# Eddie-Wang1120/Eddie-Wang-Hackathon2023

Hardware: AMD Instinct MI355X
Metric: decode tokens/s, whole job (encoder + cross-KV + language-ID + prefill + greedy decode), Whisper large-v2 int8 weight-only + int8 KV; rtf reported beside it (higher is better)
Workload: dtype f16

## Files before the change

### eddie-wang-hackathon2023_amd/csrc/attn_decode.hip

```cpp
#include <hip/hip_ext.h>

#include <atomic>

#include "common.h"
#include "kernels.h"

namespace wm {

constexpr float ATTN_SCALE = 0.35355339059327373f;
constexpr int MAX_L = 4;

template <bool I8>
__global__ __launch_bounds__(64) void attn_self_kernel(AttnSelfParams p) {
    __builtin_amdgcn_s_setprio(3);

    constexpr int MAXT = 512;
    __shared__ float s_p[MAXT];
    __shared__ h16 s_qall[MAX_L][64], s_knew[MAX_L][64], s_vnew[MAX_L][64];

    const int h = blockIdx.x, lane = threadIdx.x;
    int b = blockIdx.y;
    const int32_t* lsrc = p.live ? p.live : (const int32_t*)p.part;
    const int32_t live_n = lsrc[0], live_b = lsrc[p.live ? 1 + b : 0];
    const int32_t t_now = (p.t_dev ? p.t_dev : (const int32_t*)p.part)[0];
// ... 103 lines not shown
                            }
                        }
                    } else {
                        const half8v* kr = (const half8v*)(pastK + (size_t)j * 128);
#pragma unroll
                        for (int c = 0; c < 8; ++c) {
                            const half8v w = j0 == 0 ? __builtin_bit_cast(half8v, kpre[c]) : kr[c];
#pragma unroll
                            for (int e = 0; e < 8; ++e)
                                acc = fmaf((float)s_q[c * 8 + e], r16((float)w[e] * ATTN_SCALE), acc);
                        }
                    }
                } else {
                    const h16* kn = s_knew[j - T];
#pragma unroll 8
                    for (int e = 0; e < 64; ++e) acc = fmaf((float)s_q[e], r16((float)kn[e] * ATTN_SCALE), acc);
                }
                sc = r16(f32_as_is(acc));
            }
            if (j < MAXT) s_p[j] = sc;
            mx = fmaxf(mx, sc);
        }
        mx = wave_max_nomfma(mx);
        float sum = 0.f;
        __syncthreads();
        for (int j = lane; j < nk; j += 64) {
            const float e = __expf(s_p[j] - mx);
            s_p[j] = e;
            sum += e;
        }
        sum = wave_sum_nomfma(sum);
        const float inv = 1.0f / sum;
        __syncthreads();
        for (int j = lane; j < nk; j += 64) s_p[j] = r16(s_p[j] * inv);
        __syncthreads();
        float o = 0.f;
        int j = 0;
        if (I8) {
            const int8_t* pv = (const int8_t*)pastV + lane;
#pragma unroll
            for (int u = 0; u < 32; ++u)
                if (u < T) o = fmaf(s_p[u], r16((float)vpre8[u] * t_dq), o);
            j = min(T, 32);
            for (; j + 32 <= T; j += 32) {
                int8_t vq[32];
#pragma unroll
                for (int u = 0; u < 32; ++u) vq[u] = pv[(size_t)(j + u) * 64];
#pragma unroll
                for (int u = 0; u < 32; ++u) o = fmaf(s_p[j + u], r16((float)vq[u] * t_dq), o);
            }
            for (; j + 8 <= T; j += 8) {
                int8_t vq[8];
#pragma unroll
                for (int u = 0; u < 8; ++u) vq[u] = pv[(size_t)(j + u) * 64];
#pragma unroll
                for (int u = 0; u < 8; ++u) o = fmaf(s_p[j + u], r16((float)vq[u] * t_dq), o);
            }
            for (; j < T; ++j) o = fmaf(s_p[j], r16((float)pv[(size_t)j * 64] * t_dq), o);
        } else {
            const h16* pv = (const h16*)pastV + lane;
#pragma unroll
            for (int u = 0; u < 32; ++u)
                if (u < T) o = fmaf(s_p[u], (float)vpre16[u], o);
            j = min(T, 32);
            for (; j + 32 <= T; j += 32) {
                h16 vh[32];
#pragma unroll
                for (int u = 0; u < 32; ++u) vh[u] = pv[(size_t)(j + u) * 64];
#pragma unroll
                for (int u = 0; u < 32; ++u) o = fmaf(s_p[j + u], (float)vh[u], o);
            }
            for (; j + 8 <= T; j += 8) {
                h16 vh[8];
#pragma unroll
                for (int u = 0; u < 8; ++u) vh[u] = pv[(size_t)(j + u) * 64];
#pragma unroll
                for (int u = 0; u < 8; ++u) o = fmaf(s_p[j + u], (float)vh[u], o);
            }
            for (; j < T; ++j) o = fmaf(s_p[j], (float)pv[(size_t)j * 64], o);
        }
        for (; j < nk; ++j) o = fmaf(s_p[j], (float)s_vnew[j - T][lane], o);
        p.out[(size_t)(b * p.L + i) * p.ldo + h * 64 + lane] = (h16)f32_as_is(o);
        __syncthreads();
    }
}

constexpr int SELF_WAVES = 4;
template <bool I8>
__global__ __launch_bounds__(64 * SELF_WAVES) void attn_self_wg_kernel(AttnSelfParams p) {
    __builtin_amdgcn_s_setprio(3);
    constexpr int MAXT = 512;
    constexpr int ES = I8 ? 1 : 2;
    constexpr int ROW_B = 64 * ES;
    constexpr int DIMS = 16 / ES;
    constexpr int NCH = 64 / DIMS;
    constexpr int VROWS = 64 / NCH;
    constexpr int KCH = ROW_B / 16;
    constexpr int VPRE = 4;
    constexpr int NT = 64 * SELF_WAVES;
    __shared__ float s_p[MAXT];
    __shared__ h16 s_qall[MAX_L][64], s_knew[MAX_L][64], s_vnew[MAX_L][64];
    __shared__ float s_o[NT][DIMS + 1];
    __shared__ float s_red[2][SELF_WAVES];
    __shared__ float s_lut[I8 ? 512 + MAX_L * 64 : 1];

    const int h = blockIdx.x, tid = threadIdx.x, lane = tid & 63, wid = tid >> 6;
    int b = blockIdx.y;
    const int32_t* lsrc = p.live ? p.live : (const int32_t*)p.part;
    const int32_t live_n = lsrc[0], live_b = lsrc[p.live ? 1 + b : 0];
    const int32_t t_now = (p.t_dev ? p.t_dev : (const int32_t*)p.part)[0];
    if (p.live) {
        if (b >= live_n) return;
        b = live_b;
    }
    const int T = p.t_dev ? t_now : p.T;
    const int C = p.H * 64;
    const unsigned char* pastK = (const unsigned char*)p.past + ((size_t)b * p.past_bstride + (size_t)(0 * p.H + h) * p.past_cap * 64) * ES;
    const unsigned char* pastV = (const unsigned char*)p.past + ((size_t)b * p.past_bstride + (size_t)(1 * p.H + h) * p.past_cap * 64) * ES;
    const int vr = lane / NCH, vc = lane % NCH;
    uint4 kpre[KCH], vpre[VPRE];
    if (T > 0) {
        const int kr = min(64 * wid + lane, T - 1);
#pragma unroll
        for (int c = 0; c < KCH; ++c) kpre[c] = ((const uint4*)(pastK + (size_t)kr * ROW_B))[c];
#pragma unroll
        for (int n = 0; n < VPRE; ++n) {
            const int row = min((wid + SELF_WAVES * n) * VROWS + vr, T - 1);
            vpre[n] = *(const uint4*)(pastV + (size_t)row * ROW_B + vc * 16);
        }
    }
    const float t_dq = p.kv_scale;
    const float inv_t = 1.0f / p.kv_scale;
    if constexpr (I8) {
        const float d = r16((float)(int)(int8_t)(tid & 255) * t_dq);
        s_lut[tid & 255] = r16(d * ATTN_SCALE);
        s_lut[256 + (tid & 255)] = d;
    }
    const size_t sstride = p.part_sstride ? (size_t)p.part_sstride : (size_t)p.B * p.L * p.ldp;

    if (wid == 0) {
        for (int i = 0; i < p.L; ++i) {
            const int m = b * p.L + i;
            float q = 0.f, k = 0.f, v = 0.f;
            const h16* bsrc = p.bias ? p.bias + h * 64 + lane : (const h16*)p.part;
            const int bstep = p.bias ? C : 0;
            const h16 bq_raw = bsrc[0], bk_raw = bsrc[bstep], bv_raw = bsrc[2 * bstep];
            const float* row = p.part + (size_t)m * p.ldp + h * 64 + lane;
            int s = 0;
            for (; s + 4 <= p.ksplit; s += 4) {
                const float* r0 = row + (size_t)s * sstride;
                const float* r1 = r0 + sstride; const float* r2 = r1 + sstride; const float* r3 = r2 + sstride;
                const float q0 = r0[0], q1 = r1[0], q2 = r2[0], q3 = r3[0];
                const float k0 = r0[C], k1 = r1[C], k2 = r2[C], k3 = r3[C];
                const float v0 = r0[2 * C], v1 = r1[2 * C], v2 = r2[2 * C], v3 = r3[2 * C];
                q += (q0 + q1) + (q2 + q3); k += (k0 + k1) + (k2 + k3); v += (v0 + v1) + (v2 + v3);
            }
            for (; s < p.ksplit; ++s) {
                const float* r0 = row + (size_t)s * sstride;
                q += r0[0]; k += r0[C]; v += r0[2 * C];
            }
            q = r16(q + (p.bias ? (float)bq_raw : 0.f));
            k = r16(k + (p.bias ? (float)bk_raw : 0.f));
            v = r16(v + (p.bias ? (float)bv_raw : 0.f));
            if (p.amax) {
                const float a = wave_max_nomfma(fmaxf(fabsf(q), fmaxf(fabsf(k), fabsf(v))));
                if (lane == 0) atomicMax((unsigned int*)p.amax, __float_as_uint(a));
// ... 47 lines not shown
                            acc = fmaf((float)s_q[c * 16 + e], s_lut[idx], acc);
                        }
                    } else {
                        const half8v wh = __builtin_bit_cast(half8v, w);
                        const half8v kn8 = *(const half8v*)(&s_knew[jn][c * 8]);
#pragma unroll
                        for (int e = 0; e < 8; ++e) {
                            const float xk = cached ? (float)wh[e] : (float)kn8[e];
                            acc = fmaf((float)s_q[c * 8 + e], r16(xk * ATTN_SCALE), acc);
                        }
                    }
                }
                sc = r16(f32_as_is(acc));
                s_p[j] = sc;
            }
            mx = fmaxf(mx, sc);
        }
        mx = wave_max_nomfma(mx);
        if (lane == 0) s_red[0][wid] = mx;
        __syncthreads();
        mx = fmaxf(fmaxf(s_red[0][0], s_red[0][1]), fmaxf(s_red[0][2], s_red[0][3]));
        const float e0 = tid < nk ? __expf(s_p[tid] - mx) : 0.f;
        const float e1 = tid + NT < nk ? __expf(s_p[tid + NT] - mx) : 0.f;
        const float wsum = wave_sum_nomfma(e0 + e1);
        if (lane == 0) s_red[1][wid] = wsum;
        __syncthreads();
        const float inv = 1.0f / ((s_red[1][0] + s_red[1][1]) + (s_red[1][2] + s_red[1][3]));
        if (tid < nk) s_p[tid] = r16(e0 * inv);
        if (tid + NT < nk) s_p[tid + NT] = r16(e1 * inv);
        __syncthreads();
        float o[DIMS];
#pragma unroll
        for (int d = 0; d < DIMS; ++d) o[d] = 0.f;
        auto add_block = [&](int vb, const uint4& w) {
            const int row = vb * VROWS + vr;
            const float pj = row < T ? s_p[row] : 0.f;
            if (I8) {
                const uint32_t ws[4] = {w.x, w.y, w.z, w.w};
#pragma unroll
                for (int d = 0; d < 16; ++d)
                    o[d] = fmaf(pj, s_lut[256 + ((ws[d >> 2] >> (8 * (d & 3))) & 0xff)], o[d]);
            } else {
                const half8v wh = __builtin_bit_cast(half8v, w);
#pragma unroll
                for (int d = 0; d < 8; ++d) o[d] = fmaf(pj, (float)wh[d], o[d]);
            }
        };
#pragma unroll
        for (int n = 0; n < VPRE; ++n) {
            const int vb = wid + SELF_WAVES * n;
            if (vb * VROWS < T) add_block(vb, vpre[n]);
        }
        for (int vb = wid + SELF_WAVES * VPRE; vb * VROWS < T; vb += SELF_WAVES) {
            const int row = min(vb * VROWS + vr, T - 1);
            add_block(vb, *(const uint4*)(pastV + (size_t)row * ROW_B + vc * 16));
        }
#pragma unroll
        for (int d = 0; d < DIMS; ++d) s_o[tid][d] = o[d];
        __syncthreads();
        if (wid == 0) {
            const int ch = lane / DIMS, d = lane % DIMS;
            float part[SELF_WAVES][VROWS];
#pragma unroll
            for (int w = 0; w < SELF_WAVES; ++w)
#pragma unroll
                for (int r = 0; r < VROWS; ++r) part[w][r] = s_o[w * 64 + r * NCH + ch][d];
            float acc = 0.f;
#pragma unroll
            for (int w = 0; w < SELF_WAVES; ++w)
#pragma unroll
                for (int r = 0; r < VROWS; ++r) acc += part[w][r];
            for (int j = T; j < nk; ++j) acc = fmaf(s_p[j], (float)s_vnew[j - T][lane], acc);
            p.out[(size_t)(b * p.L + i) * p.ldo + h * 64 + lane] = (h16)f32_as_is(acc);
        }
        __syncthreads();
    }
}

int launch_attn_self(const AttnSelfParams& p, hipStream_t stream) {
    WM_REQUIRE(p.L >= 1 && p.L <= MAX_L, "attn_self: L=%d out of range [1,%d]", p.L, MAX_L);
    WM_REQUIRE(p.T + p.L <= 512, "attn_self: T+L=%d exceeds 512", p.T + p.L);
    WM_REQUIRE(p.T + p.L <= p.present_cap, "attn_self: present capacity %d < T+L=%d", p.present_cap, p.T + p.L);
    WM_REQUIRE(!p.int8_kv || p.kv_scale > 0.f, "attn_self: int8 KV needs a positive scale");
    WM_REQUIRE(p.waves == 0 || p.waves == 1 || p.waves == SELF_WAVES, "attn_self: waves=%d (0, 1 or %d)", p.waves, SELF_WAVES);
    if (p.waves == SELF_WAVES) {
        if (p.int8_kv) hipLaunchKernelGGL(attn_self_wg_kernel<true>, dim3(p.H, p.B), dim3(64 * SELF_WAVES), 0, stream, p);
        else hipLaunchKernelGGL(attn_self_wg_kernel<false>, dim3(p.H, p.B), dim3(64 * SELF_WAVES), 0, stream, p);
    } else if (p.int8_kv)
        hipLaunchKernelGGL(attn_self_kernel<true>, dim3(p.H, p.B), dim3(64), 0, stream, p);
    else
        hipLaunchKernelGGL(attn_self_kernel<false>, dim3(p.H, p.B), dim3(64), 0, stream, p);
    WM_LAUNCH_CHECK(stream, "attn_self");
    return 0;
}

constexpr int CROSS_MAX_KEYS = 1536;
constexpr int CROSS_MAX_SPLIT = 16;


template <int L, bool I8 = false, int UNR_ = 0, bool SKIP = false>
__global__ __launch_bounds__(256) void attn_cross_kernel(AttnCrossParams p) {
    constexpr int DPL = I8 ? 16 : 8;
    constexpr int LPR = 64 / DPL;
    constexpr int RPI = 64 / LPR;
    constexpr int ESZ = I8 ? 1 : 2;
#ifndef CROSS_UNR
#define CROSS_UNR 4
#endif
    constexpr int UNR = UNR_ > 0 ? UNR_ : CROSS_UNR;
    __shared__ float s_sc[L][CROSS_MAX_KEYS];
    __shared__ float s_red[L][4][2];
    __shared__ float s_o[4][L][64];
    __shared__ unsigned char s_live[SKIP ? CROSS_MAX_KEYS / 8 : 1];

    const int tid = threadIdx.x, lane = tid & 63, wid = __builtin_amdgcn_readfirstlane(tid >> 6);
    const int sub = lane % LPR, rowi = lane / LPR;
    const int per_split = (((p.Tk + p.nsplit - 1) / p.nsplit) + 7) & ~7;
    constexpr int STRIDE = 4 * RPI * UNR;
    const int first = wid * (RPI * UNR);
    const int n_rows = p.live ? p.live[0] : p.B;
    const int n_items = p.H * n_rows * p.nsplit;

    struct Item { int h, b, sp, k_begin, nkeys; const unsigned char* K; const unsigned char* V; };
    auto geometry = [&](int item) {
        Item it;
        it.h = item % p.H; it.b = (item / p.H) % n_rows; it.sp = item / (p.H * n_rows);
        if (p.live) it.b = p.live[1 + it.b];
        it.k_begin = it.sp * per_split;
        it.nkeys = max(0, min(p.Tk, it.k_begin + per_split) - it.k_begin);
        it.K = (const unsigned char*)p.kv + ((size_t)it.b * p.kv_bstride + ((size_t)(0 * p.H + it.h) * p.Tk) * 64) * ESZ;
        it.V = (const unsigned char*)p.kv + ((size_t)it.b * p.kv_bstride + ((size_t)(1 * p.H + it.h) * p.Tk) * 64) * ESZ;
        return it;
    };
    auto issue = [&](u32x4 (&dst)[UNR], const unsigned char* base, int k_begin, int nkeys, int r0) {
#pragma unroll
        for (int u = 0; u < UNR; ++u) {
            const int rr = min(r0 + u * RPI + rowi, nkeys - 1);
            dst[u] = __builtin_nontemporal_load((const u32x4*)(base + ((size_t)(k_begin + rr) * 64 + sub * DPL) * ESZ));
        }
        __builtin_amdgcn_sched_barrier(0);
    };

    auto pipeline = [&](u32x4 (&X)[UNR], u32x4 (&Y)[UNR], int nb, auto&& fetch, auto&& consume) {
        int k = 0;
        for (; k + 2 < nb; k += 2) {
            fetch(Y, k + 1);
            consume(X, k);
            fetch(X, k + 2);
            consume(Y, k + 1);
        }
        if (nb - k == 2) {
            fetch(Y, k + 1);
            consume(X, k);
            consume(Y, k + 1);
        } else {
            consume(X, k);
        }
    };
    for (int item = blockIdx.x; item < n_items; item += gridDim.x) {
    const Item it = geometry(item);
    const int h = it.h, b = it.b, sp = it.sp, k_begin = it.k_begin, nkeys = it.nkeys;
    if (nkeys == 0) {
        for (int idx = tid; idx < L * 66; idx += 256) {
            float* w = p.ws + ((((size_t)b * p.H + h) * p.nsplit + sp) * L) * 66;
            w[idx] = (idx % 66 == 0) ? -INFINITY : 0.f;
        }
        continue;
    }
    const unsigned char* K = it.K;
    const unsigned char* V = it.V;
    const int nb = (nkeys + STRIDE - 1) / STRIDE;
    u32x4 bufA[UNR], bufB[UNR];
    issue(bufA, K, k_begin, nkeys, first);

// ... 361 lines not shown
```

### eddie-wang-hackathon2023_amd/csrc/engine.hip

```cpp
#include <stdarg.h>
#include <stdio.h>
#include <stdlib.h>
#include <string.h>

#include <atomic>
#include <map>
#include <mutex>
#include <unordered_map>
#include <string>
#include <vector>

#include "../../include/whisper_mi355.h"
#include "common.h"
#include "kernels.h"

namespace wm {

static thread_local char g_err[1024] = "";
void set_error(const char* fmt, ...) {
    va_list ap;
    va_start(ap, fmt);
    vsnprintf(g_err, sizeof(g_err), fmt, ap);
    va_end(ap);
}
// ... 558 lines not shown
}
}

namespace { constexpr int DEC_CHUNK = 4; }

size_t wm_decoder_workspace_bytes(const wm_engine* e, int batch, int n_new) {
    if (!e || e->kind != WM_ENGINE_DECODER || batch < 1 || n_new < 1) return 0;
    if (n_new <= DEC_CHUNK) return carve_decoder(e, batch, n_new, nullptr).total;
    return carve_decoder(e, batch, DEC_CHUNK, nullptr).total + align_up((size_t)batch * DEC_CHUNK * e->dims.n_vocab * sizeof(h16));
}

namespace {
__global__ void stamp_kernel(long long* tl, int cap, long long tag, long long what) {
    if (threadIdx.x != 0) return;
    const int i = atomicAdd((int*)tl, 1);
    if (i < cap) { tl[1 + 3 * i] = tag; tl[2 + 3 * i] = what; tl[3 + 3 * i] = wall_clock64(); }
}

constexpr int SMALL_PATH_DEFAULT_ROWS = 16;
std::atomic<int> g_cross_v_skip{CROSS_V_SKIP_DEFAULT};
std::atomic<int> g_decode_chain{DECODE_CHAIN_DEFAULT};
struct ChainDev {
    std::mutex mu;
    int n_cu = 0;
    unsigned* err_host = nullptr; unsigned* err_dev = nullptr;
    bool declined = false; std::string reason, footprint;
    std::map<long long, bool> resident;
    std::atomic<long long> launches{0};
    std::atomic<long long> declined_calls{0};
};
ChainDev g_chain_dev[64];
static ChainDev& chain_dev_slot(int device) { return g_chain_dev[device >= 0 && device < 64 ? device : 0]; }
int chain_dev_init(ChainDev& cd, int device) {
    std::lock_guard<std::mutex> lk(cd.mu);
    if (cd.n_cu > 0 && cd.err_host) return 0;
    int v = 0;
    WM_CHECK_HIP(hipDeviceGetAttribute(&v, hipDeviceAttributeMultiprocessorCount, device));
    void* host = nullptr; void* dev = nullptr;
    WM_CHECK_HIP(hipHostMalloc(&host, 64, hipHostMallocMapped | hipHostMallocCoherent));
    memset(host, 0, 64);
    WM_CHECK_HIP(hipHostGetDevicePointer(&dev, host, 0));
    cd.err_host = (unsigned*)host; cd.err_dev = (unsigned*)dev;
    cd.n_cu = v > 0 ? v : 1;
    return 0;
}
inline unsigned chain_err_peek(const ChainDev& cd) {
    return cd.err_host ? __atomic_load_n(cd.err_host, __ATOMIC_RELAXED) : 0u;
}
bool stream_has_all_cus(hipStream_t s, int n_cu) {
    uint32_t mask[32];
    memset(mask, 0, sizeof(mask));
    if (hipExtStreamGetCUMask(s, 32, mask) != hipSuccess) { (void)hipGetLastError(); return true; }
    int bits = 0;
    for (uint32_t m : mask) bits += __builtin_popcount(m);
    return bits == 0 || bits >= n_cu;
}
std::atomic<int> g_small_rows{-1};
int small_path_max_rows() {
    int r = g_small_rows.load(std::memory_order_relaxed);
    if (r < 0) {
        r = lab_env_int("WM_SMALL_PATH", SMALL_PATH_DEFAULT_ROWS);
        r = r < 0 ? 0 : (r > GEMV_SMALL_MAX_M ? GEMV_SMALL_MAX_M : r);
        g_small_rows.store(r, std::memory_order_relaxed);
    }
    return r;
}

std::atomic<int> g_rows_min{-1};
int rows_path_min_rows() {
    int r = g_rows_min.load(std::memory_order_relaxed);
    if (r < 0) {
        r = lab_env_int("WM_ROWS_PATH", 1) == 0 ? 0 : lab_env_int("WM_ROWS_MIN", 40);
        if (r < 0) r = 0;
        g_rows_min.store(r, std::memory_order_relaxed);
    }
    return r;
}

std::atomic<int> g_self_waves{-1};
int self_attn_waves(int rows) {
    int w = g_self_waves.load(std::memory_order_relaxed);
    if (w < 0) {
        w = lab_env_int("WM_SELF_WAVES", 0);
        if (w != 1 && w != 4) w = 0;
        g_self_waves.store(w, std::memory_order_relaxed);
    }
    return w ? w : (rows <= small_path_max_rows() ? 4 : 1);
}

int chain_max_rows() {
    static const int r = [] { const int v = lab_env_int("WM_CHAIN_ROWS", CHAIN_MAX_ROWS); return v < 1 ? 1 : (v > CHAIN_MAX_ROWS ? CHAIN_MAX_ROWS : v); }();
    return r;
}

struct GroupStep {
    const wm_engine* e; const wm_decoder_io* io; DecWs w;
    int B, L, T, C, H, M;
    bool small = false;
    bool chain = false;
    int chain_wgs = 0; unsigned* chain_err = nullptr; ChainDev* chain_cd = nullptr;
    bool rows = false;
    bool fused() const { return small || rows; }

    int gemv(const Lin& l, const h16* A, int lda, int mode, const h16* ln_g, const h16* ln_b, h16* out16, int ld16, hipStream_t s) {
        GemvSmallParams p{};
        p.A = A; p.lda = lda; p.M = M; p.K = l.K; p.Wt = l.w; p.n_blocks = l.n_blocks; p.w8 = l.wcode; p.scale = l.s;
        p.ln_g = ln_g; p.ln_b = ln_b;
        p.mode = mode; p.bias = l.b; p.gelu_kind = e->gelu();
        p.out32 = w.part; p.ld32 = l.N;
        p.out16 = out16; p.ld16 = ld16; p.n_valid = l.N;
        p.x = w.x; p.ldx = C;
        return small ? launch_gemv_small(p, s) : launch_gemm_rows(p, s);
    }

    Profiler* prof = nullptr;

    void mark(int layer, int pos, hipStream_t s) {
        static const bool fine = lab_env_int("WM_TIMELINE_FINE", 0) == 1;
        if (fine && prof->timeline)
            hipLaunchKernelGGL(stamp_kernel, dim3(1), dim3(64), 0, s, prof->timeline, prof->timeline_cap, (long long)(uintptr_t)io->logits, (long long)(1000 + 32 * layer + pos));
    }

    int init(const wm_engine* e_, const wm_decoder_io* io_, hipStream_t stream, bool alone = true) {
        e = e_; io = io_;
        prof = &g_prof_dev[e->device >= 0 && e->device < MAX_DEVICES ? e->device : 0];
        WM_REQUIRE(io && io->tokens && io->positional_embedding && io->present && io->cross && io->logits && io->workspace,
                   "wm_decoder_step: null argument");
        const wm_dims& d = e->dims;
        B = io->batch; L = io->n_new; T = io->n_past; C = d.n_text_state; H = d.n_text_head; M = B * L;
        WM_REQUIRE(B >= 1 && L >= 1 && L <= 4 && T >= 0, "wm_decoder_step: bad batch/n_new/n_past (%d, %d, %d)", B, L, T);
        WM_REQUIRE(T + L <= d.n_text_ctx, "wm_decoder_step: T+L=%d exceeds n_text_ctx=%d", T + L, d.n_text_ctx);
        WM_REQUIRE(T == 0 || io->past, "wm_decoder_step: n_past > 0 needs past buffers");
        WM_REQUIRE(T == 0 || io->past_capacity >= T, "wm_decoder_step: past capacity %d < n_past %d", io->past_capacity, T);
        WM_REQUIRE(io->present_capacity >= T + L, "wm_decoder_step: present capacity %d < n_past + n_new = %d", io->present_capacity, T + L);
        WM_REQUIRE(!io->n_past_dev || (L == 1 && io->past), "wm_decoder_step: a device step counter needs n_new == 1 and past buffers");
        WM_REQUIRE(C == H * 64, "head size must be 64");
        w = carve_decoder(e, B, L, io->workspace);
        WM_REQUIRE(io->workspace_bytes >= w.total, "decoder workspace too small: %zu < %zu", io->workspace_bytes, w.total);
        small = M <= small_path_max_rows();
        rows = !small && rows_path_min_rows() > 0 && M >= rows_path_min_rows() && !e->dec.empty() && gemm_rows_supports(C, e->dec[0].qkv.wcode);
        chain = false;
        hipStreamCaptureStatus cap_st = hipStreamCaptureStatusNone;
        const bool capturing = hipStreamIsCapturing(stream, &cap_st) == hipSuccess && cap_st != hipStreamCaptureStatusNone;
        ChainDev& cd = chain_dev_slot(e->device);
        if (!capturing && chain_err_peek(cd) != 0) {
            set_error("wm_decoder_step: a one-launch decode step on device %d gave up waiting for its workgroups (they were not resident "
                      "together): the results since then are invalid.  Call wm_decode_chain_error() to acknowledge and decode again -- the device "
                      "takes the launch-per-kernel path from then on (wm_set_decode_chain re-arms the one-launch forms)", e->device);
            return 1;
        }
        if (alone && small && L == 1 && M <= chain_max_rows() && !e->dec.empty() && e->chain_dev && g_decode_chain.load(std::memory_order_relaxed) && !io->qkv_amax) {
            if (chain_dev_init(cd, e->device)) return 2;
            const int n_cu = cd.n_cu;
            chain_wgs = n_cu > 256 ? 256 : n_cu; chain_err = cd.err_dev; chain_cd = &cd;
            bool ok = gemv_chain_supports(C, e->dec[0].qkv.wcode, n_cu) && w.nsplit == 4 && !e->i8cross() && self_attn_waves(M) == 4 &&
                      io->present_capacity <= 512 && !(M > 2 && e->dec[0].qkv.wcode == 4) &&
                      (M > 4 ? (M * H <= chain_wgs && M * H * w.nsplit <= 4 * chain_wgs)
                             : M * H + (M > 2 ? (M * H * w.nsplit + 1) / 2 : M * H * w.nsplit) <= chain_wgs);
            for (int i = 0; ok && i < e->dims.n_text_layer; ++i)
                ok = io->present[i] && io->cross[i] &&
                     (T == 0 ? io->n_past_dev == nullptr : (io->past[i] == io->present[i] && io->past_capacity == io->present_capacity));
            if (ok) {
                std::lock_guard<std::mutex> lk(cd.mu);
                ok = !cd.declined;
                if (ok) {
                    const long long key = ((long long)M << 48) | ((long long)e->dec[0].qkv.wcode << 40) | ((long long)(e->i8kv() ? 1 : 0) << 32) | ((long long)e->dims.n_audio_ctx << 8) | w.nsplit;
                    auto it = cd.resident.find(key);
// ... 401 lines not shown
}

int wm_step_advance(int32_t* counter, wm_stream_t stream) { return launch_step_advance(counter, (hipStream_t)stream); }
int wm_step_finish(int32_t* counter, const int32_t* done, int batch, int32_t* live, wm_stream_t stream) {
    return launch_step_finish(counter, done, batch, live, (hipStream_t)stream);
}

int wm_gemm(const void* A, int lda, int M, int K, const void* W, int N, int w8, const void* scale,
            const void* bias, const void* residual, int ldr, int act, void* C, int ldc,
            void* workspace, size_t workspace_bytes, wm_stream_t stream) {
    GemmBigParams p{};
    p.A = (const h16*)A; p.lda = lda; p.M = M; p.K = K; p.W = W; p.N = N;
    p.bias = (const h16*)bias; p.C = (h16*)C; p.ldc = ldc;
    p.residual = (const h16*)residual; p.ldr = ldr; p.act = act;
    if (w8) {
        WM_REQUIRE(scale && workspace, "wm_gemm: int8 weights need their scales and a workspace for the fp16 expansion");
        WM_REQUIRE(workspace_bytes >= (size_t)N * K * sizeof(h16), "wm_gemm: workspace too small: %zu < %zu", workspace_bytes, (size_t)N * K * sizeof(h16));
        if (launch_dequant_w8((const int8_t*)W, (const h16*)scale, (h16*)workspace, N, K, (hipStream_t)stream)) return 2;
        p.W = workspace;
    }
    return launch_gemm_f16(p, (hipStream_t)stream);
}

int wm_conv1d_gelu(const void* x_pad, int B, int T_in, int C_in, const void* W, int K, const void* bias, int C_out,
                   int stride, int gelu, void* out, wm_stream_t stream) {
    WM_REQUIRE(x_pad && W && out && B >= 1 && T_in >= 1, "wm_conv1d_gelu: null argument or empty input");
    WM_REQUIRE(stride == 1 || stride == 2, "wm_conv1d_gelu: stride %d (1 or 2)", stride);
    WM_REQUIRE(T_in % stride == 0 && K >= 3 * C_in, "wm_conv1d_gelu: T_in=%d, K=%d < 3*C_in=%d", T_in, K, 3 * C_in);
    const int T_out = T_in / stride;
    GemmBigParams p{};
    p.A = (const h16*)x_pad; p.lda = stride * C_in; p.M = B * T_out; p.K = K; p.W = W; p.N = C_out;
    p.a_rows = T_out; p.a_bstride = (long)(T_in + 2) * C_in;
    p.bias = (const h16*)bias; p.C = (h16*)out; p.ldc = C_out; p.act = gelu;
    return launch_gemm_f16(p, (hipStream_t)stream);
}

int wm_argmax(const void* logits, int64_t row_stride, int batch, int n_vocab, int32_t* ids, wm_stream_t stream) {
    WM_REQUIRE(logits && ids && batch >= 1 && n_vocab >= 1, "wm_argmax: null argument or empty input");
    return launch_argmax((const h16*)logits, (long)row_stride, batch, n_vocab, ids, (hipStream_t)stream);
}

int wm_gemm_skinny(const void* A, int lda, int M, int K, const void* Wt, int n_blocks, int w8,
                   const void* scale, int ksplit, float* part, wm_stream_t stream) {
    GemmSkinnyParams p{};
    p.A = (const h16*)A; p.lda = lda; p.M = M; p.K = K; p.Wt = Wt; p.n_blocks = n_blocks; p.w8 = w8;
    p.scale = (const h16*)scale; p.ksplit = ksplit; p.part = part;
    return launch_gemm_skinny(p, (hipStream_t)stream);
}
int wm_gemm_skinny_default_ksplit(int M, int K, int n_blocks, int w8) { return skinny_default_ksplit(M, K, n_blocks, w8); }

int wm_set_rows_path(int min_rows) {
    const int prev = rows_path_min_rows();
    g_rows_min.store(min_rows < 0 ? 0 : min_rows, std::memory_order_relaxed);
    return prev;
}

int wm_gemm_rows(const wm_gemv_io* io, wm_stream_t stream) {
    WM_REQUIRE(io && io->a && io->wt, "wm_gemm_rows: null argument");
    GemvSmallParams p{};
    p.A = (const h16*)io->a; p.lda = io->lda; p.M = io->m; p.K = io->k; p.Wt = io->wt; p.n_blocks = io->n_blocks; p.w8 = io->w8;
    p.scale = (const h16*)io->scale;
    p.ln_g = (const h16*)io->ln_gamma; p.ln_b = (const h16*)io->ln_beta;
    p.mode = io->mode; p.bias = (const h16*)io->bias; p.gelu_kind = io->gelu_kind;
    p.out32 = io->out32; p.ld32 = io->ld32; p.out16 = (h16*)io->out16; p.ld16 = io->ld16; p.n_valid = io->n_valid;
    p.x = (h16*)io->x; p.ldx = io->ldx;
    return launch_gemm_rows(p, (hipStream_t)stream);
}

int wm_lab_knobs(char* buf, size_t cap) {
    std::lock_guard<std::mutex> lk(g_lab_mu);
    if (buf && cap > 0) { strncpy(buf, g_lab_honoured.c_str(), cap - 1); buf[cap - 1] = 0; }
    return (int)g_lab_honoured.size();
}

int wm_set_gemm_small_tiles(int tiles) {
    const int prev = get_gemm_small_tiles();
    set_gemm_small_tiles(tiles);
    return prev;
}

int wm_set_self_attn_waves(int waves) {
    self_attn_waves(1);
    const int prev = g_self_waves.load(std::memory_order_relaxed);
    g_self_waves.store(waves == 1 || waves == 4 ? waves : 0, std::memory_order_relaxed);
    return prev;
}

int wm_set_small_batch_rows(int rows) {
    const int prev = small_path_max_rows();
    g_small_rows.store(rows < 0 ? 0 : (rows > GEMV_SMALL_MAX_M ? GEMV_SMALL_MAX_M : rows), std::memory_order_relaxed);
    return prev;
}

int wm_gemv_fused(const wm_gemv_io* io, wm_stream_t stream) {
    WM_REQUIRE(io && io->a && io->wt, "wm_gemv_fused: null argument");
    GemvSmallParams p{};
    p.A = (const h16*)io->a; p.lda = io->lda; p.M = io->m; p.K = io->k; p.Wt = io->wt; p.n_blocks = io->n_blocks; p.w8 = io->w8;
    p.scale = (const h16*)io->scale;
    p.ln_g = (const h16*)io->ln_gamma; p.ln_b = (const h16*)io->ln_beta;
    p.mode = io->mode; p.bias = (const h16*)io->bias; p.gelu_kind = io->gelu_kind;
    p.out32 = io->out32; p.ld32 = io->ld32; p.out16 = (h16*)io->out16; p.ld16 = io->ld16; p.n_valid = io->n_valid;
    p.x = (h16*)io->x; p.ldx = io->ldx;
    return launch_gemv_small(p, (hipStream_t)stream);
}

int wm_layernorm(const void* x, int ldx, int M, int N, const void* gamma, const void* beta, void* out, int ldo,
                 wm_stream_t stream) {
    return launch_layernorm((const h16*)x, ldx, M, N, (const h16*)gamma, (const h16*)beta, (h16*)out, ldo, (hipStream_t)stream);
}

int wm_attn_encoder(const void* qkv, int ld, int B, int T, int H, void* out, int ldo, wm_stream_t stream) {
    AttnEncParams p{(const h16*)qkv, ld, B, T, H, (h16*)out, ldo};
    return launch_attn_encoder(p, (hipStream_t)stream);
}

int wm_attn_decode_cross(const float* q, int B, int L, int H, int Tk, const void* kv, void* out, int nsplit,
                         float* ws, wm_stream_t stream) {
    AttnCrossParams p{};
    p.part = q; p.ksplit = 1; p.ldp = H * 64; p.bias = nullptr;
    p.B = B; p.L = L; p.H = H; p.Tk = Tk; p.kv = (const h16*)kv; p.kv_bstride = (long)2 * H * Tk * 64;
    p.out = (h16*)out; p.ldo = H * 64; p.nsplit = nsplit; p.ws = ws;
    p.skip_zero_rows = g_cross_v_skip.load(std::memory_order_relaxed);
    return launch_attn_cross(p, (hipStream_t)stream);
}

int wm_set_decode_chain(int on) {
    const int prev = g_decode_chain.load(std::memory_order_relaxed);
    g_decode_chain.store(on < 0 ? DECODE_CHAIN_DEFAULT : (on > 2 ? 2 : on), std::memory_order_relaxed);
    for (ChainDev& cd : g_chain_dev) {
        std::lock_guard<std::mutex> lk(cd.mu);
        if (cd.declined) { cd.declined = false; cd.reason.clear(); }
    }
    return prev;
}

int wm_decode_chain_error(int* out) {
    WM_REQUIRE(out, "wm_decode_chain_error: null argument");
    ChainDev& cd = chain_dev_slot(current_device_index());
    const unsigned v = chain_err_peek(cd);
    *out = (int)v;
    if (v) {
        std::lock_guard<std::mutex> lk(cd.mu);
        __atomic_store_n(cd.err_host, 0u, __ATOMIC_RELAXED);
        cd.declined = true;
        cd.reason = "a one-launch decode step gave up waiting for its workgroups (they were not resident together)";
    }
    return 0;
}

int wm_decode_chain_status(wm_chain_status* out) {
    WM_REQUIRE(out, "wm_decode_chain_status: null argument");
    ChainDev& cd = chain_dev_slot(current_device_index());
    std::lock_guard<std::mutex> lk(cd.mu);
    memset(out, 0, sizeof(*out));
    out->mode = g_decode_chain.load(std::memory_order_relaxed);
    out->launches = cd.launches.load(std::memory_order_relaxed);
    out->declined_calls = cd.declined_calls.load(std::memory_order_relaxed);
    out->declined = cd.declined ? 1 : 0;
    out->error_pending = chain_err_peek(cd) ? 1 : 0;
    snprintf(out->reason, sizeof(out->reason), "%s", cd.reason.c_str());
    snprintf(out->footprint, sizeof(out->footprint), "%s", cd.footprint.c_str());
    return 0;
}

int wm_debug_occupy(int n_workgroups, size_t lds_bytes, int64_t microseconds, wm_stream_t stream) {
    return launch_occupy(n_workgroups, lds_bytes, (long long)microseconds, (hipStream_t)stream);
}
// ... 47 lines not shown
```

### eddie-wang-hackathon2023_amd/csrc/kernels.h

```cpp
#pragma once
#include "common.h"

namespace wm {

struct GemmBigParams {
    const h16* A; int lda; int M; int K;
    const void* W; int N;
    const h16* bias;
    h16* C; int ldc;
    const h16* residual; int ldr; int res_mod;
    int act;
    int colscale_n; float colscale;
    int out_mode;
    int hs_T, hs_H, hs_kv;
    float q8_inv_scale;
    int a_rows; long a_bstride;
    int c_rows; long c_bstride;
    int max_wgs;
    int nt_flags;
    int tile_rows;
};
int launch_gemm_f16(const GemmBigParams& p, hipStream_t stream);
constexpr int GEMM_SMALL_TILES_DEFAULT = 150;
constexpr int GEMM_TINY_TILES_DEFAULT = 160;
// ... 43 lines not shown
};
struct ChainLayerStatic { const h16* qkv_bias; const h16* cq_bias; float kv_scale; int pad_; };
struct ChainLayerIo { const void* cross_kv; void* cache; };
struct GemvChainParams {
    int n_stages; const ChainStage* st;
    float* out32;
    int w8, gelu_kind;
    h16* x;
    unsigned long long* gran_x; unsigned long long* gran_h;
    const h16* cross_kv; int cross_Tk, cross_heads, cross_nsplit; const h16* cross_qbias;
    unsigned long long* gran_q;
    int cross_at, merge_at, merge_nsplit, merge_heads;
    unsigned long long* gran_p;
    const float* self_part; const h16* self_bias; void* self_cache; int self_cap, self_T, self_heads, self_i8; const int32_t* self_t_dev;
    float self_kv_scale; h16* self_out; unsigned long long* gran_c;
    int n_layers; const ChainLayerStatic* lstat; const ChainLayerIo* lio; unsigned long long* gran_s;
    int rows; long cross_row_bytes, self_row_bytes;
    const int32_t* live;
    unsigned* err;
    const unsigned* generation; int launch_id;
};
bool gemv_chain_supports(int C, int w8, int n_cu);
int gemv_chain_resident(int w8, int self_i8, int rows, int cross_Tk, int cross_nsplit, int n_wg, int n_cu, bool* ok, char* why, size_t why_cap);
int launch_occupy(int n_wg, size_t lds_bytes, long long usec, hipStream_t stream);
int launch_gemv_chain(const GemvChainParams& p, const ChainStage* host_stages, int n_wg, hipStream_t stream);
int launch_chain_io_table(ChainLayerIo* dst, const ChainLayerIo* host, int n, hipStream_t stream);

bool gemm_rows_supports(int K, int w8);
int launch_gemm_rows(const GemvSmallParams& p, hipStream_t stream);

struct RowFinishParams {
    const float* part; int ksplit; int M; int N; int ldp;
    long part_sstride;
    const h16* bias;
    int mode; int gelu_kind;
    h16* x; int ldx;
    const h16* ln_g; const h16* ln_b;
    h16* out; int ldo;
    int eager;
};
int launch_row_finish(const RowFinishParams& p, hipStream_t stream);

struct EmbedParams {
    const int32_t* tokens; int tokens_ld;
    int M;
    int L;
    const void* emb_tiles; int C;
    const h16* pos;
    h16* x; int ldx;
    int n_vocab;
    const int32_t* t_dev;
    unsigned* generation;
};
int launch_embed(const EmbedParams& p, hipStream_t stream);

int launch_mel_transpose_pad(const h16* mel, int B, int n_mels, int T, h16* out ,
                             hipStream_t stream);
int launch_zero_pad_rows(h16* buf, int B, int Tpad, int C, hipStream_t stream);
int launch_layernorm(const h16* x, int ldx, int M, int N, const h16* g, const h16* b, h16* out, int ldo,
                     hipStream_t stream);

struct AttnEncParams {
    const h16* qkv; int ld;
    int B, T, H;
    h16* out; int ldo;
    int max_wgs;
};
int launch_attn_encoder(const AttnEncParams& p, hipStream_t stream);

struct AttnSelfParams {
    const float* part; int ksplit; int ldp;
    long part_sstride;
    const h16* bias;
    int B, L, T, H;
    const void* past; long past_bstride; int past_cap;
    void* present; long present_bstride; int present_cap;
    int int8_kv; float kv_scale;
    float* amax;
    const int32_t* t_dev;
    h16* out; int ldo;
    const int32_t* live;
    int waves;
};
int launch_attn_self(const AttnSelfParams& p, hipStream_t stream);

struct AttnCrossParams {
    const float* part; int ksplit; int ldp;
    long part_sstride;
    const h16* bias;
    int B, L, H, Tk;
    const h16* kv; long kv_bstride;
    float kv_q8_scale;
    h16* out; int ldo;
    int nsplit;
    float* ws;
    const int32_t* live;
    int skip_zero_rows;
};
constexpr int CROSS_V_SKIP_DEFAULT = 1;
int launch_attn_cross(const AttnCrossParams& p, hipStream_t stream, hipEvent_t ev_start = nullptr, hipEvent_t ev_stop = nullptr);

struct GreedyParams {
    h16* logits; long ld_row;
    int B; int V;
    int32_t* tokens; int ld_tok; int cur_len;
    float* sum_logprobs;
    const int32_t* suppress; int n_suppress;
    const int32_t* blank; int n_blank;
    int sample_begin; int eot; int timestamp_begin; int max_initial_ts;
    int apply_rules;
    int32_t* n_done;
    const int32_t* t_dev;
    int32_t* done;
    const int32_t* row_limit;
    float temperature;
    uint32_t seed_lo, seed_hi; const uint32_t* seed_dev;
    int row0;
};
int launch_greedy(const GreedyParams& p, hipStream_t stream);
int launch_step_advance(int32_t* counter, hipStream_t stream);
int launch_step_finish(int32_t* counter, const int32_t* done, int B, int32_t* live, hipStream_t stream);
int launch_argmax(const h16* logits, long ld_row, int B, int V, int32_t* ids, hipStream_t stream);

constexpr int BEAM_MAX = 8, BEAM_POOL_MAX = 16;
struct BeamCand { float lp; int32_t tok; };
struct BeamParams {
    GreedyParams g;
    int K, max_cand, ignore_eot;
    int32_t* parent;
    int32_t* fin_tokens; float* fin_scores; int32_t* fin_len; int32_t* fin_count;
    int32_t* live_len;
    BeamCand* cand;
};
int launch_beam_step(const BeamParams& p, hipStream_t stream);
struct KvReorderParams {
    void* const* layers; int n_layer, rows, K, H, cap, elem_bytes;
    const int32_t* parent; const int32_t* done; int n_last; const int32_t* t_dev;
};
int launch_kv_reorder(const KvReorderParams& p, hipStream_t stream);

size_t log_mel_workspace_bytes(int batch, int n_samples, int n_mels);
int launch_log_mel(const float* audio, int batch, int n_samples, long audio_ld, const float* filters, int n_mels,
                   h16* out16, float* out32, void* workspace, size_t workspace_bytes, hipStream_t stream);

int launch_quantize_i8(const h16* x, int8_t* q, long n, float inv_scale, hipStream_t stream);

}
```

Baseline: 16650.

## Add multi-head-per-block self-attention kernel for large decode batches

Adds a new self-attention decode kernel that packs four heads per 256-thread block. All threads share the key-score work across the heads, and the V rows are staged through LDS with double-buffered prefetch. For int8 KV it adds an LDS lookup table for dequantisation, and it specialises on L==1 and priority. It replaces the old one-wave-per-head path used when waves==1, which is the default for larger row counts, and keeps the legacy kernel behind a new waves value. The aim is better occupancy and load spreading when there are many rows, at the cost of more LDS per block and extra code complexity.

```diff
diff --git a/eddie-wang-hackathon2023_amd/csrc/attn_decode.hip b/eddie-wang-hackathon2023_amd/csrc/attn_decode.hip
--- a/eddie-wang-hackathon2023_amd/csrc/attn_decode.hip
+++ b/eddie-wang-hackathon2023_amd/csrc/attn_decode.hip
@@ -209,6 +209,265 @@
         for (; j < nk; ++j) o = fmaf(s_p[j], (float)s_vnew[j - T][lane], o);
         p.out[(size_t)(b * p.L + i) * p.ldo + h * 64 + lane] = (h16)f32_as_is(o);
         __syncthreads();
+    }
+}
+
+constexpr int ROWS_HEADS = 4;
+__device__ __forceinline__ void wave_lds_sync() {
+    __builtin_amdgcn_fence(__ATOMIC_RELEASE, "wavefront");
+    __builtin_amdgcn_wave_barrier();
+    __builtin_amdgcn_fence(__ATOMIC_ACQUIRE, "wavefront");
+}
+template <bool I8, bool PRIO, bool ONE>
+__global__ __launch_bounds__(64 * ROWS_HEADS, ONE ? 4 : 2) void attn_self_rows_kernel(AttnSelfParams p) {
+    if (PRIO) __builtin_amdgcn_s_setprio(3);
+    constexpr int MAXT = 512;
+    constexpr int ES = I8 ? 1 : 2;
+    constexpr int ROW_B = 64 * ES;
+    constexpr int KCH = ROW_B / 16;
+    constexpr int VROWS = 64 / KCH;
+    constexpr int VLD = 4;
+    constexpr int BLK = VLD * VROWS;
+    constexpr int NT = 64 * ROWS_HEADS;
+    __shared__ float s_p[ROWS_HEADS][MAXT];
+    __shared__ h16 s_q[ROWS_HEADS][MAX_L][64], s_kf[ROWS_HEADS][MAX_L][64], s_vnew[ROWS_HEADS][MAX_L][64];
+    __shared__ u32x4 s_v[ROWS_HEADS][VLD * 64];
+    __shared__ float s_lut[I8 ? 512 : 1];
+
+    const int tid = threadIdx.x, lane = tid & 63, wid = __builtin_amdgcn_readfirstlane(tid >> 6);
+    const int h0 = blockIdx.x * ROWS_HEADS, nh = min(ROWS_HEADS, p.H - h0);
+    const int h = h0 + wid;
+    const bool active = wid < nh;
+    int b = blockIdx.y;
+    const int32_t* lsrc = p.live ? p.live : (const int32_t*)p.part;
+    const int32_t live_n = lsrc[0], live_b = lsrc[p.live ? 1 + b : 0];
+    const int32_t t_now = (p.t_dev ? p.t_dev : (const int32_t*)p.part)[0];
+    if (p.live) {
+        if (b >= live_n) return;
+        b = live_b;
+    }
+    const int T = __builtin_amdgcn_readfirstlane(p.t_dev ? t_now : p.T);
+    const int C = p.H * 64;
+    const int L = ONE ? 1 : p.L;
+    const unsigned char* pastB = (const unsigned char*)p.past + (size_t)b * p.past_bstride * ES;
+    const size_t head_b = (size_t)p.past_cap * ROW_B;
+    const unsigned char* pastV = pastB + (size_t)(p.H + h) * head_b;
+    const int npairs = nh * T;
+    auto pair_of = [&](int g, int Tt, int& hh, int& j) {
+        hh = (g >= Tt) + (g >= 2 * Tt) + (g >= 3 * Tt);
+        j = g - hh * Tt;
+    };
+    u32x4 kpre[KCH], vb[VLD];
+    int hh0 = 0, j0 = 0;
+    auto fetch_v = [&](int blk, int Tt, int ln) {
+#pragma unroll
+        for (int n = 0; n < VLD; ++n) {
+            const int row = min(blk * BLK + n * VROWS + ln / KCH, Tt - 1);
+            vb[n] = *(const u32x4*)(pastV + (size_t)row * ROW_B + (ln % KCH) * 16);
+        }
+    };
+    auto stage_v = [&](int ln) {
+#pragma unroll
+        for (int n = 0; n < VLD; ++n) s_v[wid][n * 64 + ln] = vb[n];
+    };
+    if (T > 0) {
+        pair_of(min(tid, npairs - 1), T, hh0, j0);
+        const unsigned char* kr = pastB + (size_t)(h0 + hh0) * head_b + (size_t)j0 * ROW_B;
+#pragma unroll
+        for (int c = 0; c < KCH; ++c) kpre[c] = ((const u32x4*)kr)[c];
+        if (active) fetch_v(0, T, lane);
+    }
+    const float t_dq = p.kv_scale;
+    const float inv_t = 1.0f / p.kv_scale;
+    if constexpr (I8) {
+        const float d = r16((float)(int)(int8_t)(tid & 255) * t_dq);
+        s_lut[tid & 255] = r16(d * ATTN_SCALE);
+        s_lut[256 + (tid & 255)] = d;
+    }
+    const size_t sstride = p.part_sstride ? (size_t)p.part_sstride : (size_t)p.B * L * p.ldp;
+    const int nblk = (T + BLK - 1) / BLK;
+
+    if (active) {
+        for (int i = 0; i < L; ++i) {
+            const int m = b * L + i;
+            float q = 0.f, k = 0.f, v = 0.f;
+            const h16* bsrc = p.bias ? p.bias + h * 64 + lane : (const h16*)p.part;
+            const int bstep = p.bias ? C : 0;
+            const h16 bq_raw = bsrc[0], bk_raw = bsrc[bstep], bv_raw = bsrc[2 * bstep];
+            const float* row = p.part + (size_t)m * p.ldp + h * 64 + lane;
+            int s = 0;
+            for (; s + 4 <= p.ksplit; s += 4) {
+                const float* r0 = row + (size_t)s * sstride;
+                const float* r1 = r0 + sstride; const float* r2 = r1 + sstride; const float* r3 = r2 + sstride;
+                const float q0 = r0[0], q1 = r1[0], q2 = r2[0], q3 = r3[0];
+                const float k0 = r0[C], k1 = r1[C], k2 = r2[C], k3 = r3[C];
+                const float v0 = r0[2 * C], v1 = r1[2 * C], v2 = r2[2 * C], v3 = r3[2 * C];
+                q += (q0 + q1) + (q2 + q3); k += (k0 + k1) + (k2 + k3); v += (v0 + v1) + (v2 + v3);
+            }
+            for (; s < p.ksplit; ++s) {
+                const float* r0 = row + (size_t)s * sstride;
+                q += r0[0]; k += r0[C]; v += r0[2 * C];
+            }
+            q = r16(q + (p.bias ? (float)bq_raw : 0.f));
+            k = r16(k + (p.bias ? (float)bk_raw : 0.f));
+            v = r16(v + (p.bias ? (float)bv_raw : 0.f));
+            if (p.amax) {
+                const float a = wave_max_nomfma(fmaxf(fabsf(q), fmaxf(fabsf(k), fabsf(v))));
+                if (lane == 0) atomicMax((unsigned int*)p.amax, __float_as_uint(a));
+            }
+            s_kf[wid][i][lane] = (h16)r16(k * ATTN_SCALE);
+            s_vnew[wid][i][lane] = (h16)v;
+            const size_t off_k = (size_t)b * p.present_bstride + ((size_t)(0 * p.H + h) * p.present_cap + T + i) * 64 + lane;
+            const size_t off_v = (size_t)b * p.present_bstride + ((size_t)(1 * p.H + h) * p.present_cap + T + i) * 64 + lane;
+            if (I8) {
+                ((int8_t*)p.present)[off_k] = (int8_t)fminf(127.f, fmaxf(-128.f, rintf(k * inv_t)));
+                ((int8_t*)p.present)[off_v] = (int8_t)fminf(127.f, fmaxf(-128.f, rintf(v * inv_t)));
+            } else {
+                ((h16*)p.present)[off_k] = (h16)k;
+                ((h16*)p.present)[off_v] = (h16)v;
+            }
+            s_q[wid][i][lane] = (h16)r16(q * ATTN_SCALE);
+        }
+        const bool inplace = (p.past == p.present) && (p.past_cap == p.present_cap) && (p.past_bstride == p.present_bstride);
+        if (!inplace && T > 0) {
+            for (int kv = 0; kv < 2; ++kv) {
+                const unsigned char* src = (const unsigned char*)p.past + ((size_t)b * p.past_bstride + (size_t)(kv * p.H + h) * p.past_cap * 64) * ES;
+                unsigned char* dst = (unsigned char*)p.present + ((size_t)b * p.present_bstride + (size_t)(kv * p.H + h) * p.present_cap * 64) * ES;
+                const int n16 = T * 64 * ES / 16;
+                for (int c = lane; c < n16; c += 64) ((uint4*)dst)[c] = ((const uint4*)src)[c];
+            }
+        }
+        if (T > 0) {
+            stage_v(lane);
+            if (nblk > 1) fetch_v(1, T, lane);
+        }
+    }
+    __syncthreads();
+
+    auto score = [&](const u32x4 (&w)[KCH], int hh, int j, int i) {
+        const h16* sq = s_q[hh][i];
+        float acc = 0.f;
+        if constexpr (I8) {
+            float f[2][8];
+            auto lookup = [&](int c, float (&dst)[8]) {
+                const uint32_t ws[4] = {w[c >> 1].x, w[c >> 1].y, w[c >> 1].z, w[c >> 1].w};
+#pragma unroll
+                for (int e = 0; e < 8; ++e) dst[e] = s_lut[(ws[(c & 1) * 2 + (e >> 2)] >> (8 * (e & 3))) & 0xff];
+            };
+            half8v qa[2];
+            lookup(0, f[0]);
+            qa[0] = *(const half8v*)sq;
+#pragma unroll
+            for (int c = 0; c < 2 * KCH; ++c) {
+                if (c + 1 < 2 * KCH) {
+                    lookup(c + 1, f[(c + 1) & 1]);
+                    qa[(c + 1) & 1] = *(const half8v*)(sq + (c + 1) * 8);
+                }
+                __builtin_amdgcn_sched_barrier(0);
+#pragma unroll
+                for (int e = 0; e < 8; ++e) acc = fmaf((float)qa[c & 1][e], f[c & 1][e], acc);
+                asm volatile("" : "+v"(acc) : : "memory");
+                __builtin_amdgcn_sched_barrier(0);
+            }
+        } else {
+#pragma unroll
+            for (int c = 0; c < KCH; ++c) {
+                const half8v wh = __builtin_bit_cast(half8v, w[c]);
+                const half8v qa = *(const half8v*)(sq + c * 8);
+#pragma unroll
+                for (int e = 0; e < 8; ++e) acc = fmaf((float)qa[e], r16((float)wh[e] * ATTN_SCALE), acc);
+                if (c & 1) __builtin_amdgcn_sched_barrier(0);
+            }
+        }
+        if (j < MAXT) s_p[hh][j] = r16(f32_as_is(acc));
+    };
+
+    int lds_blk = 0;
+    for (int i = 0; i < L; ++i) {
+        int Ti = T, ln = lane;
+        if (!ONE) {
+            asm volatile("" : "+s"(Ti));
+            asm volatile("" : "+v"(ln));
+        }
+        const int tn = wid * 64 + ln, np = nh * Ti, nb = (Ti + BLK - 1) / BLK;
+        const int nk = Ti + i + 1;
+        if (i > 0 && Ti > 0) {
+            const unsigned char* kr = pastB + (size_t)(h0 + hh0) * head_b + (size_t)j0 * ROW_B;
+#pragma unroll
+            for (int c = 0; c < KCH; ++c) kpre[c] = ((const u32x4*)kr)[c];
+        }
+        if (tn < np) score(kpre, hh0, j0, i);
+        for (int g = tn + NT; g < np; g += NT) {
+            int hh, j;
+            pair_of(g, Ti, hh, j);
+            const unsigned char* kr = pastB + (size_t)(h0 + hh) * head_b + (size_t)j * ROW_B;
+            u32x4 w[KCH];
+#pragma unroll
+            for (int c = 0; c < KCH; ++c) w[c] = ((const u32x4*)kr)[c];
+            score(w, hh, j, i);
+        }
+        if (active && ln <= i) {
+            const h16* sq = s_q[wid][i];
+            const h16* kf = s_kf[wid][ln];
+            float acc = 0.f;
+#pragma unroll 8
+            for (int e = 0; e < 64; ++e) acc = fmaf((float)sq[e], (float)kf[e], acc);
+            if (Ti + ln < MAXT) s_p[wid][Ti + ln] = r16(f32_as_is(acc));
+        }
+        __syncthreads();
+        if (active) {
+            float* sp = s_p[wid];
+            float mx = -INFINITY;
+            for (int j = ln; j < nk; j += 64) mx = fmaxf(mx, sp[j]);
+            mx = wave_max_nomfma(mx);
+            float sum = 0.f;
+            for (int j = ln; j < nk; j += 64) {
+                const float e = __expf(sp[j] - mx);
+                sp[j] = e;
+                sum += e;
+            }
+            sum = wave_sum_nomfma(sum);
+            const float inv = 1.0f / sum;
+            for (int j = ln; j < nk; j += 64) sp[j] = r16(sp[j] * inv);
+            wave_lds_sync();
+            if (lds_blk != 0) {
+                fetch_v(0, Ti, ln);
+                wave_lds_sync();
+                stage_v(ln);
+                if (nb > 1) fetch_v(1, Ti, ln);
+                wave_lds_sync();
+                lds_blk = 0;
+            }
+            float o = 0.f;
+            auto vrow = [&](int u) -> float {
+                if constexpr (I8) return s_lut[256 + ((const unsigned char*)s_v[wid])[u * 64 + ln]];
+                else return (float)((const h16*)s_v[wid])[u * 64 + ln];
+            };
+            for (int blk = 0; blk < nb; ++blk) {
+                const int j0b = blk * BLK, n = min(BLK, Ti - j0b);
+                int u = 0;
+                for (; u + 8 <= n; u += 8) {
+                    const float4 pa = *(const float4*)(sp + j0b + u), pb = *(const float4*)(sp + j0b + u + 4);
+                    const float pj[8] = {pa.x, pa.y, pa.z, pa.w, pb.x, pb.y, pb.z, pb.w};
+                    float vv[8];
+#pragma unroll
+                    for (int r = 0; r < 8; ++r) vv[r] = vrow(u + r);
+#pragma unroll
+                    for (int r = 0; r < 8; ++r) o = fmaf(pj[r], vv[r], o);
+                }
+                for (; u < n; ++u) o = fmaf(sp[j0b + u], vrow(u), o);
+                if (blk + 1 < nb) {
+                    wave_lds_sync();
+                    stage_v(ln);
+                    if (blk + 2 < nb) fetch_v(blk + 2, Ti, ln);
+                    wave_lds_sync();
+                    lds_blk = blk + 1;
+                }
+            }
+            for (int j = Ti; j < nk; ++j) o = fmaf(sp[j], (float)s_vnew[wid][j - Ti][ln], o);
+            p.out[(size_t)(b * L + i) * p.ldo + h * 64 + ln] = (h16)f32_as_is(o);
+        }
+        if (i + 1 < L) __syncthreads();
     }
 }
 
@@ -422,14 +681,30 @@
     WM_REQUIRE(p.T + p.L <= 512, "attn_self: T+L=%d exceeds 512", p.T + p.L);
     WM_REQUIRE(p.T + p.L <= p.present_cap, "attn_self: present capacity %d < T+L=%d", p.present_cap, p.T + p.L);
     WM_REQUIRE(!p.int8_kv || p.kv_scale > 0.f, "attn_self: int8 KV needs a positive scale");
-    WM_REQUIRE(p.waves == 0 || p.waves == 1 || p.waves == SELF_WAVES, "attn_self: waves=%d (0, 1 or %d)", p.waves, SELF_WAVES);
+    WM_REQUIRE(p.waves == 0 || p.waves == 1 || p.waves == SELF_WAVES || p.waves == SELF_WAVES_LEGACY, "attn_self: waves=%d (0, 1, %d or %d)", p.waves,
+               SELF_WAVES, SELF_WAVES_LEGACY);
     if (p.waves == SELF_WAVES) {
         if (p.int8_kv) hipLaunchKernelGGL(attn_self_wg_kernel<true>, dim3(p.H, p.B), dim3(64 * SELF_WAVES), 0, stream, p);
         else hipLaunchKernelGGL(attn_self_wg_kernel<false>, dim3(p.H, p.B), dim3(64 * SELF_WAVES), 0, stream, p);
-    } else if (p.int8_kv)
-        hipLaunchKernelGGL(attn_self_kernel<true>, dim3(p.H, p.B), dim3(64), 0, stream, p);
-    else
-        hipLaunchKernelGGL(attn_self_kernel<false>, dim3(p.H, p.B), dim3(64), 0, stream, p);
+    } else if (p.waves == SELF_WAVES_LEGACY) {
+        if (p.int8_kv) hipLaunchKernelGGL(attn_self_kernel<true>, dim3(p.H, p.B), dim3(64), 0, stream, p);
+        else hipLaunchKernelGGL(attn_self_kernel<false>, dim3(p.H, p.B), dim3(64), 0, stream, p);
+    } else {
+        static const int prio = lab_env_int("WM_SELF_PRIO", 1);
+        const dim3 grid((p.H + ROWS_HEADS - 1) / ROWS_HEADS, p.B), block(64 * ROWS_HEADS);
+        auto go = [&](auto kernel) { hipLaunchKernelGGL(kernel, grid, block, 0, stream, p); };
+        const int pick = (p.int8_kv ? 4 : 0) | (prio ? 2 : 0) | (p.L == 1 ? 1 : 0);
+        switch (pick) {
+            case 0: go(attn_self_rows_kernel<false, false, false>); break;
+            case 1: go(attn_self_rows_kernel<false, false, true>); break;
+            case 2: go(attn_self_rows_kernel<false, true, false>); break;
+            case 3: go(attn_self_rows_kernel<false, true, true>); break;
+            case 4: go(attn_self_rows_kernel<true, false, false>); break;
+            case 5: go(attn_self_rows_kernel<true, false, true>); break;
+            case 6: go(attn_self_rows_kernel<true, true, false>); break;
+            default: go(attn_self_rows_kernel<true, true, true>); break;
+        }
+    }
     WM_LAUNCH_CHECK(stream, "attn_self");
     return 0;
 }
diff --git a/eddie-wang-hackathon2023_amd/csrc/engine.hip b/eddie-wang-hackathon2023_amd/csrc/engine.hip
--- a/eddie-wang-hackathon2023_amd/csrc/engine.hip
+++ b/eddie-wang-hackathon2023_amd/csrc/engine.hip
@@ -664,7 +664,7 @@
     int w = g_self_waves.load(std::memory_order_relaxed);
     if (w < 0) {
         w = lab_env_int("WM_SELF_WAVES", 0);
-        if (w != 1 && w != 4) w = 0;
+        if (w != 1 && w != 4 && w != SELF_WAVES_LEGACY) w = 0;
         g_self_waves.store(w, std::memory_order_relaxed);
     }
     return w ? w : (rows <= small_path_max_rows() ? 4 : 1);
@@ -1232,7 +1232,7 @@
 int wm_set_self_attn_waves(int waves) {
     self_attn_waves(1);
     const int prev = g_self_waves.load(std::memory_order_relaxed);
-    g_self_waves.store(waves == 1 || waves == 4 ? waves : 0, std::memory_order_relaxed);
+    g_self_waves.store(waves == 1 || waves == 4 || waves == SELF_WAVES_LEGACY ? waves : 0, std::memory_order_relaxed);
     return prev;
 }
 
diff --git a/eddie-wang-hackathon2023_amd/csrc/kernels.h b/eddie-wang-hackathon2023_amd/csrc/kernels.h
--- a/eddie-wang-hackathon2023_amd/csrc/kernels.h
+++ b/eddie-wang-hackathon2023_amd/csrc/kernels.h
@@ -149,6 +149,7 @@
     const int32_t* live;
     int waves;
 };
+constexpr int SELF_WAVES_LEGACY = 64;
 int launch_attn_self(const AttnSelfParams& p, hipStream_t stream);
 
 struct AttnCrossParams {
```

After: 16800 (median of 6 runs). Within noise of the previous version (+0.9%).
